# JiawangBian/SC-SfMLearner-Release

Hardware: AMD Instinct MI355X
Metric: train images/sec (+ warp-loss ms/step) KITTI 256x832 RN18 (higher is better)
Workload: dtype f32; 1 GPU; configs[1]: kitti 256x832, batch 12/GPU, 2 refs (seq 3), ResNet18 DispNet + ResNet18 PoseNet, ssim+mask+auto-mask, zeros padding, 1 scale; global_batch=12, parallelism=1 GPU, memory_format=contiguous (NCHW)

## Files before the change

### __graft_entry__.py

```python
import os
import sys

ROOT = os.path.dirname(os.path.abspath(__file__))
PKG = os.path.join(ROOT, "sc-sfmlearner-release_amd")
for p in (ROOT, PKG):
    if p not in sys.path:
        sys.path.insert(0, p)


REPORT_ORDER = ("dgrad", "vlog", "wrw", "decb", "enceval", "val", "dvis", "", "nets", "eval", "odom", "enc", "stem", "snip",
                "vis", "prep")


def build() -> None:
    from scsfm_hip import _lib, build as hip_build
    from scsfm_hip.libraries import BY_NAME, LATER, NEWER, ROWS
    libs = {row.name: _lib.CLib(hip_build.build_lib(row.name, force=False), row.header, row.abi, row.prefix)
            for row in ROWS}
    assert libs[""]._dll.scsfm_abi_version() == _lib.ABI_VERSION
    import inverse_warp
    import loss_functions
    import models
    from scsfm_hip import decoder, depth_eval, depth_vis, encoder, odometry, prepare, snippets, visualise
    from scsfm_hip import conv_wrw, decoder_bias, decoder_dgrad, encoder_eval, validation, validation_log
    from scsfm_hip import encoder_frozen, optim, training_state
    from oracle import scsfm_oracle
    for row in NEWER:
        print(f"[{row.tag}] {libs[row.name].path}: {len(libs[row.name].decls)} entry points resolved (ABI {row.abi})")
    for name in tuple(row.name for row in LATER) + REPORT_ORDER:
        print(f"[{BY_NAME[name].tag}] {libs[name].path}: {len(libs[name].decls)} entry points resolved")


def smoke() -> None:
    import torch

    import loss_functions as LF
    from oracle import scsfm_oracle as O
    from scsfm_hip import _lib, synth

    assert torch.cuda.is_available(), "smoke() needs a HIP device"
    lib = _lib.get()
    assert lib.path.endswith("libscsfm_hip.so")
    dev = torch.device("cuda:0")
    d = synth.make_batch(2, 128, 416, n_ref=2, seed=0, depth="smooth")

    def leaves(device):
        mv = lambda t: t.to(device).clone().requires_grad_(True)
        return ([mv(t) for t in d["tgt_depth"]], [[mv(t) for t in r] for r in d["ref_depths"]],
                [mv(p) for p in d["poses"]], [mv(p) for p in d["poses_inv"]])

    td, rd, ps, pi = leaves(dev)
    tgt, refs, K = d["tgt_img"].to(dev), [r.to(dev) for r in d["ref_imgs"]], d["intrinsics"].to(dev)
    photo, geom = LF.compute_photo_and_geometry_loss(tgt, refs, K, td, rd, ps, pi, 1, 1, 1, 1, "zeros")
    smooth = LF.compute_smooth_loss(td, tgt, rd, refs)
    (photo + 0.1 * smooth + 0.5 * geom).backward()
    torch.cuda.synchronize()

    td_c, rd_c, ps_c, pi_c = leaves("cpu")
    photo_c, geom_c = O.photo_and_geometry_loss(d["tgt_img"], d["ref_imgs"], d["intrinsics"], td_c, rd_c, ps_c, pi_c,
                                                1, 1, 1, 1, "zeros")
    smooth_c = O.smooth_loss(td_c, d["tgt_img"], rd_c, d["ref_imgs"])
    (photo_c + 0.1 * smooth_c + 0.5 * geom_c).backward()
    for name, a, b in (("photo", photo, photo_c), ("geom", geom, geom_c), ("smooth", smooth, smooth_c)):
        err = abs(float(a) - float(b))
        print(f"[smoke] {name}: hip {float(a):.7f} oracle {float(b):.7f} |d| {err:.2e}")
        assert err <= 1e-5, name
    pairs = [("g_tgt_depth", td[0].grad, td_c[0].grad), ("g_ref0_depth", rd[0][0].grad, rd_c[0][0].grad),
             ("g_ref1_depth", rd[1][0].grad, rd_c[1][0].grad), ("g_pose0", ps[0].grad, ps_c[0].grad),
             ("g_pose_inv1", pi[1].grad, pi_c[1].grad)]
    for name, a, b in pairs:
        scale = float(b.abs().max())
        bad = ((a.cpu() - b).abs() > 0.01 * scale).double().mean().item()
        print(f"[smoke] {name}: scale {scale:.3e} share of entries off by >1% of scale {bad:.2e}")
        assert bad <= 2e-3, name
    import torch.nn as nn
    from scsfm_hip import encoder as E
    assert _lib.get_stem().path.endswith("libscsfm_stem.so")
    xs = torch.randn(2, 4, 6, 8, device=dev)
    bn_a, bn_b = nn.BatchNorm2d(4).to(dev).train(), nn.BatchNorm2d(4).to(dev).train()
    f0, pooled = E.bn_act(xs, bn_a, pool=True)
    f0_ref = E.bn_act(xs, bn_b)
    assert torch.equal(f0, f0_ref) and torch.equal(pooled, E.max_pool(f0_ref))
    print("[smoke] stem: fused BatchNorm / ReLU / max-pool equals the separate ops")
    import numpy as np
    from scsfm_hip import visualise as V
    assert _lib.get_vis().path.endswith("libscsfm_vis.so")
    ramp = torch.linspace(0.05, 12.0, 70).reshape(2, 5, 7)
    for cmap, max_value in (("bone", None), ("rainbow", 10)):
        got = V.colourise(ramp.to(dev), colormap=cmap, max_value=max_value).cpu().numpy()
        table = V.colour_table(cmap)
        r = ramp.numpy()
        d = r.reshape(2, -1).max(axis=1)[:, None, None] if max_value is None else np.float32(max_value)
        xa = (r / d).astype(np.float32) * np.float32(len(table))
        want = table[np.clip(xa.astype(np.int64), 0, len(table) - 1)]
        assert got.shape == (2, 5, 7, 4) and np.array_equal(got, want), cmap
    print("[smoke] vis: bone and rainbow pictures of a ramp equal the table lookup")
    from scsfm_hip import depth_vis as DV
    assert _lib.get_dvis().path.endswith("libscsfm_dvis.so")
    depth = torch.linspace(0.5, 80.0, 35).reshape(5, 7)
    rng_, pics = DV.depth_pictures([depth.to(dev)])
    inv = 1 / (depth.numpy() + np.float32(1e-6))
    vmin, vmax = float(inv.min()), float(np.percentile(inv, 95))
    assert rng_.cpu().numpy().tolist() == [[vmin, vmax]]
    v = ((inv.astype(np.float64) - vmin).astype(np.float32).astype(np.float64) / (vmax - vmin)).astype(np.float32)
    xa = v * np.float32(256)
    want = DV.MAGMA[np.where(xa >= 256, 255, np.clip(xa, 0, 255).astype(np.int64))]
    assert pics[0].shape == (5, 7, 3) and np.array_equal(pics[0].cpu().numpy(), want)
    print("[smoke] dvis: the magma picture of a depth ramp equals the table lookup")
    from scsfm_hip import validation as VA
    assert _lib.get_val().path.endswith("libscsfm_val.so")
    f32 = np.float32
    rng = np.random.default_rng(0)
    gt_v = rng.uniform(0.05, 90.0, (2, 20, 60)).astype(f32)
    disp_v = rng.uniform(0.01, 1.5, (2, 10, 30)).astype(f32)
    res = VA.depth_errors(torch.from_numpy(gt_v).to(dev), torch.from_numpy(disp_v).to(dev), "kitti", is_disp=True)
    got = VA.batch_mean(res)
    y1, y2, x1, x2 = int(0.40810811 * 20), int(0.99189189 * 20), int(0.03594771 * 60), int(0.96405229 * 60)
    want = np.zeros(6)
    for g, dsp in zip(gt_v, disp_v):
        p = (f32(1) / dsp)[np.arange(20) // 2][:, np.arange(60) // 2]
        ok = np.zeros((20, 60), bool)
        ok[y1:y2, x1:x2] = True
        ok &= (g > f32(0.1)) & (g < f32(80))
        g, p = g[ok], np.clip(p[ok], f32(1e-3), f32(80))
        p = p * np.sort(g)[(g.size - 1) // 2] / np.sort(p)[(p.size - 1) // 2]
        t = np.maximum(g / p, p / g)
        e = np.abs(g - p).astype(np.float64)
        want += [e.mean(), (e / g).mean(), (e * e / g).mean(), (t < 1.25).mean(), (t < 1.25 ** 2).mean(),
                 (t < 1.25 ** 3).mean()]
    want /= 2
    print(f"[smoke] val: abs_rel hip {got[1]:.7f} numpy {want[1]:.7f}; a1 hip {got[3]:.7f} numpy {want[3]:.7f}")
    assert res.count.cpu().numpy().min() > 100 and np.allclose(got, want, rtol=1e-6, atol=0), (got, want)
    table = VA.ValidationTable(4, dev)
    rows_v = [(0.25, 0.002, 1.5), (0.5, float("nan"), 0.75), (0.125, 0.004, 0.25)]
    for i, vals_v in zip((0, 1, 3), rows_v):
        table.add_losses(i, *torch.tensor(vals_v, device=dev))
    mean_v, n_v = table.finish()
    sums_v = [0.0] * 4
    for p_v, s_v, g_v in rows_v:
        sums_v = [a + float(f32(b)) for a, b in zip(sums_v, (p_v, p_v, s_v, g_v))]
    want_v = [s / 3 for s in sums_v] + [0.0] * 3
    print(f"[smoke] val: table of 3 present rows of 4: photo {mean_v[1]:.7f} host {want_v[1]:.7f}, smooth {mean_v[2]} "
          f"(a NaN row), geometry {mean_v[3]:.7f} host {want_v[3]:.7f}")
    assert n_v == 3 and np.isnan(mean_v[2]) and mean_v[:2] + mean_v[3:] == want_v[:2] + want_v[3:], (mean_v, want_v)
    import torch.nn.functional as F
    from scsfm_hip import encoder_eval as EE
    assert _lib.get_enceval().path.endswith("libscsfm_enceval.so")
    bn_e = nn.BatchNorm2d(4).to(dev)
    with torch.no_grad():
        bn_e.running_mean.copy_(torch.tensor([0.5, -1.0, 0.0, 2.0]))
        bn_e.running_var.copy_(torch.tensor([0.25, 1.0, 4.0, 0.5]))
        bn_e.weight.copy_(torch.tensor([1.0, -0.5, 2.0, 0.0]))
        bn_e.bias.copy_(torch.tensor([0.0, 0.1, -0.2, 0.3]))
    bn_e.eval()
    with torch.no_grad():
        f0_e, pooled_e = EE.bn_act(xs, bn_e, pool=True)
        want_e = F.relu(bn_e(xs))
        assert torch.equal(f0_e, EE.bn_act(xs, bn_e)) and torch.equal(pooled_e, F.max_pool2d(f0_e, 3, 2, 1))
        assert torch.equal(pooled_e, EE.max_pool(f0_e))
    err_e = float((f0_e - want_e).abs().max())
    print(f"[smoke] enceval: eval-mode BatchNorm / ReLU / max-pool, max |fused - ATen| {err_e:.2e}")
    assert err_e <= 1e-5
    from scsfm_hip import decoder_bias as DB
    assert _lib.get_decb().path.endswith("libscsfm_decb.so")
    conv_b = nn.Conv2d(4, 3, 3).to(dev)
    xb = torch.randn(2, 4, 9, 11, device=dev)
    want_b = F.pad(F.elu(conv_b(xb)), (1, 1, 1, 1), mode="reflect")
    want_h = 10 * torch.sigmoid(conv_b(xb)) + 0.01
    (want_b.sum() + want_h.sum()).backward()
    want_gb = conv_b.bias.grad.clone()
    conv_b.bias.grad = None
    raw = F.conv2d(xb, conv_b.weight, None)
    got_b, got_h = DB.elu_pad(raw, conv_b.bias), DB.disp_head(raw, conv_b.bias, 10, 0.01)
    (got_b.sum() + got_h.sum()).backward()
    err_b = float((conv_b.bias.grad - want_gb).abs().max() / want_gb.abs().max())
    print(f"[smoke] decb: bias folded into elu_pad and disp_head, relative bias-gradient difference {err_b:.2e}")
    assert torch.equal(got_b, want_b) and float((got_h - want_h).abs().max()) <= 1e-6 and err_b <= 1e-5
    _smoke_wrw(dev)
    _smoke_vlog(dev)
    _smoke_dgrad(dev)
    _smoke_fbn(dev)
    _smoke_opt(dev)
    print("[smoke] ok")


def _smoke_opt(dev) -> None:
    import numpy as np
    import torch

    from scsfm_hip import _lib
    from scsfm_hip import optim as OP
    assert _lib.get_opt().path.endswith("libscsfm_opt.so")
    f32 = np.float32
    g = torch.Generator().manual_seed(7)
    shapes, lrs, wd, betas, eps = ((7,), (4, 6), (2 * OP.CHUNK + 3,), (3, 5, 5)), (1e-3, 1e-2), 0.01, (0.9, 0.999), 1e-8
    host = [torch.randn(s, generator=g) for s in shapes]
    params = [torch.nn.Parameter(t.to(dev)) for t in host]
    opt = OP.Adam([{"params": params[:2], "lr": lrs[0]}, {"params": params[2:], "lr": lrs[1]}], betas=betas, eps=eps,
                  weight_decay=wd)
    p = [t.numpy().copy() for t in host]
    m, v = [np.zeros_like(a) for a in p], [np.zeros_like(a) for a in p]
    b1c, b2, b2c, e, w = f32(1.0 - betas[0]), f32(betas[1]), f32(1.0 - betas[1]), f32(eps), f32(wd)
    for step in (1, 2, 3):
        grads = [torch.randn(s, generator=g) for s in shapes]
        for q, gr in zip(params, grads):
            q.grad = gr.to(dev)
        opt.step()
        for k, gr in enumerate(grads):
            step_size = f32(lrs[k // 2] / (1 - betas[0] ** step))
            bc2_sqrt = f32((1 - betas[1] ** step) ** 0.5)
            gk = gr.numpy() + w * p[k]
            m[k] = m[k] + b1c * (gk - m[k])
            v[k] = v[k] * b2 + (b2c * gk) * gk
            p[k] = p[k] - step_size * (m[k] / (np.sqrt(v[k]) / bc2_sqrt + e))
    state = opt.state_dict()["state"]
    for k in range(4):
        assert p[k].dtype == f32 and torch.equal(params[k].detach().cpu(), torch.from_numpy(p[k])), k
        assert torch.equal(state[k]["exp_avg"].cpu(), torch.from_numpy(m[k])), k
        assert torch.equal(state[k]["exp_avg_sq"].cpu(), torch.from_numpy(v[k])), k
        assert float(state[k]["step"]) == 3.0
    print("[smoke] opt: three Adam steps of four tensors in one launch each equal the numpy restatement bit for bit")


def _smoke_fbn(dev) -> None:
    import torch
    import torch.nn as nn
    import torch.nn.functional as F

    from scsfm_hip import _lib
    from scsfm_hip import encoder_frozen as EF
    assert _lib.get_fbn().path.endswith("libscsfm_fbn.so")
    g = torch.Generator().manual_seed(5)
    bn = nn.BatchNorm2d(4).to(dev)
    with torch.no_grad():
        bn.running_mean.copy_(torch.tensor([0.5, -1.0, 0.0, 2.0]))
        bn.running_var.copy_(torch.tensor([0.25, 1.0, 4.0, 0.5]))
        bn.weight.copy_(torch.tensor([1.0, -0.5, 2.0, 0.25]))
        bn.bias.copy_(torch.tensor([0.0, 0.1, -0.2, 0.3]))
    assert EF.freeze(bn) == 1 and not bn.train().training
    buffers = [b.clone() for b in bn.buffers()]
    x, identity = (torch.randn(2, 4, 6, 8, generator=g).to(dev).requires_grad_(True) for _ in range(2))
    gy = torch.randn(2, 4, 6, 8, generator=g).to(dev)
    leaves = (x, identity, bn.weight, bn.bias)
    y = EF.bn_act(x, bn, identity)
    got = torch.autograd.grad(y, leaves, gy)
    y_ref = F.relu(bn(x) + identity)
    want = torch.autograd.grad(y_ref, leaves, gy)
    err_y = float((y - y_ref).abs().max())
    err = max(float((a - b).abs().max() / b.abs().max()) for a, b in zip(got, want))
    print(f"[smoke] fbn: frozen BatchNorm / add / ReLU, max |fused - ATen| {err_y:.2e}, largest relative gradient "
          f"difference {err:.2e}")
    assert err_y <= 1e-5 and err <= 1e-5
    assert all(torch.equal(a, b) for a, b in zip(buffers, bn.buffers()))


def _smoke_wrw(dev) -> None:
    import torch
    import torch.nn.functional as F

    from scsfm_hip import _lib
    from scsfm_hip import conv_wrw as CW
    assert _lib.get_wrw().path.endswith("libscsfm_wrw.so")
    xw = torch.randn(2, 16, 7, 69, device=dev, requires_grad=True)
    ww = torch.randn(16, 16, 3, 3, device=dev, requires_grad=True)
    gy = torch.randn(2, 16, 5, 67, device=dev)
    gx_w, gw_w = torch.autograd.grad(CW.conv3x3_valid(xw, ww), (xw, ww), gy)
# ... 72 lines not shown
```

### sc-sfmlearner-release_amd/models/PoseResNet.py

```python
from __future__ import absolute_import, division, print_function

import torch
import torch.nn as nn

from .resnet_encoder import ResnetEncoder


class PoseDecoder(nn.Module):
    def __init__(self, num_ch_enc, num_input_features=1, num_frames_to_predict_for=1, stride=1):
        super().__init__()
        self.net = nn.ModuleList([
            nn.Conv2d(int(num_ch_enc[-1]), 256, 1),
            nn.Conv2d(num_input_features * 256, 256, 3, stride, 1),
            nn.Conv2d(256, 256, 3, stride, 1),
            nn.Conv2d(256, 6 * num_frames_to_predict_for, 1)])
        self.relu = nn.ReLU()

    def forward(self, input_features):
        out = torch.cat([self.relu(self.net[0](f[-1])) for f in input_features], 1)
        out = self.relu(self.net[1](out))
        out = self.relu(self.net[2](out))
        out = self.net[3](out)
        return 0.01 * out.mean(3).mean(2).view(-1, 6)


class PoseResNet(nn.Module):
    def __init__(self, num_layers=18, pretrained=True):
        super().__init__()
        self.encoder = ResnetEncoder(num_layers=num_layers, pretrained=pretrained, num_input_images=2)
        self.decoder = PoseDecoder(self.encoder.num_ch_enc)

    def init_weights(self):
        pass

    def forward(self, img1, img2):
        return self.decoder([self.encoder(torch.cat([img1, img2], 1))])
```

### sc-sfmlearner-release_amd/models/resnet_encoder.py

```python
from __future__ import absolute_import, division, print_function

import numpy as np
import torch
import torch.nn as nn


_encoder_ops = None


def _E():
    global _encoder_ops
    if _encoder_ops is None:
        from scsfm_hip import encoder
        _encoder_ops = encoder
    return _encoder_ops


_encoder_eval_ops = None


def _EV():
    global _encoder_eval_ops
    if _encoder_eval_ops is None:
        from scsfm_hip import encoder_eval
        _encoder_eval_ops = encoder_eval
    return _encoder_eval_ops


_encoder_frozen_ops = None


def _EF():
    global _encoder_frozen_ops
    if _encoder_frozen_ops is None:
        from scsfm_hip import encoder_frozen
        _encoder_frozen_ops = encoder_frozen
    return _encoder_frozen_ops


def _fused_applies(x, *bns):
    return x.is_cuda and _E().applies(x, *bns)


def _eval_applies(x, *bns):
    return x.is_cuda and _EV().applies(x, *bns)


def _frozen_applies(x, *bns, relu=True):
    return x.is_cuda and not any(bn.training for bn in bns) and _EF().applies(x, *bns, relu=relu)


def _bn_act(x, bn, act, identity=None):
    if _fused_applies(x, bn) and (identity is None or _fused_applies(identity)):
        return _E().bn_act(x, bn, identity, relu=act is not None)
    if _frozen_applies(x, bn, relu=act is not None) and (identity is None or _frozen_applies(identity)):
        return _EF().bn_act(x, bn, identity, relu=act is not None)
    if _eval_applies(x, bn) and (identity is None or _eval_applies(identity)):
        return _EV().bn_act(x, bn, identity, relu=act is not None)
    out = bn(x)
    if identity is not None:
        out = out + identity
    return out if act is None else act(out)


def _downsample(ds, x):
    return _bn_act(ds[0](x), ds[1], None)


def _conv3x3(cin, cout, stride=1):
    return nn.Conv2d(cin, cout, kernel_size=3, stride=stride, padding=1, bias=False)


class BasicBlock(nn.Module):
    expansion = 1

    def __init__(self, inplanes, planes, stride=1, downsample=None):
        super().__init__()
        self.conv1 = _conv3x3(inplanes, planes, stride)
        self.bn1 = nn.BatchNorm2d(planes)
        self.relu = nn.ReLU(inplace=True)
        self.conv2 = _conv3x3(planes, planes)
        self.bn2 = nn.BatchNorm2d(planes)
        self.downsample = downsample

    def forward(self, x):
        identity = x if self.downsample is None else _downsample(self.downsample, x)
        out = _bn_act(self.conv1(x), self.bn1, self.relu)
        return _bn_act(self.conv2(out), self.bn2, self.relu, identity)

    def forward_reference(self, x):
        identity = x if self.downsample is None else self.downsample(x)
        out = self.relu(self.bn1(self.conv1(x)))
        out = self.bn2(self.conv2(out))
        return self.relu(out + identity)


class Bottleneck(nn.Module):
    expansion = 4

    def __init__(self, inplanes, planes, stride=1, downsample=None):
        super().__init__()
        self.conv1 = nn.Conv2d(inplanes, planes, kernel_size=1, bias=False)
        self.bn1 = nn.BatchNorm2d(planes)
        self.conv2 = _conv3x3(planes, planes, stride)
        self.bn2 = nn.BatchNorm2d(planes)
        self.conv3 = nn.Conv2d(planes, planes * 4, kernel_size=1, bias=False)
        self.bn3 = nn.BatchNorm2d(planes * 4)
        self.relu = nn.ReLU(inplace=True)
        self.downsample = downsample

    def forward(self, x):
        identity = x if self.downsample is None else _downsample(self.downsample, x)
        out = _bn_act(self.conv1(x), self.bn1, self.relu)
        out = _bn_act(self.conv2(out), self.bn2, self.relu)
        return _bn_act(self.conv3(out), self.bn3, self.relu, identity)

    def forward_reference(self, x):
        identity = x if self.downsample is None else self.downsample(x)
        out = self.relu(self.bn1(self.conv1(x)))
        out = self.relu(self.bn2(self.conv2(out)))
        out = self.bn3(self.conv3(out))
        return self.relu(out + identity)


class ResNet(nn.Module):

    def __init__(self, block, layers, num_classes=1000, num_input_images=1):
        super().__init__()
        self.inplanes = 64
        self.conv1 = nn.Conv2d(num_input_images * 3, 64, kernel_size=7, stride=2, padding=3, bias=False)
        self.bn1 = nn.BatchNorm2d(64)
        self.relu = nn.ReLU(inplace=True)
        self.maxpool = nn.MaxPool2d(kernel_size=3, stride=2, padding=1)
        self.layer1 = self._make_layer(block, 64, layers[0])
        self.layer2 = self._make_layer(block, 128, layers[1], stride=2)
        self.layer3 = self._make_layer(block, 256, layers[2], stride=2)
        self.layer4 = self._make_layer(block, 512, layers[3], stride=2)
        self.avgpool = nn.AdaptiveAvgPool2d((1, 1))
        self.fc = nn.Linear(512 * block.expansion, num_classes)
        for m in self.modules():
            if isinstance(m, nn.Conv2d):
                nn.init.kaiming_normal_(m.weight, mode='fan_out', nonlinearity='relu')
            elif isinstance(m, nn.BatchNorm2d):
                nn.init.constant_(m.weight, 1)
                nn.init.constant_(m.bias, 0)

    def _make_layer(self, block, planes, blocks, stride=1):
        downsample = None
        if stride != 1 or self.inplanes != planes * block.expansion:
# ... 78 lines not shown
```

### sc-sfmlearner-release_amd/scsfm_hip/_lib.py

```python
from __future__ import annotations

import ctypes
import os
import re
import threading

import torch

from .libraries import BY_NAME, HERE, LATER, ROWS, SUMMARY, TABLE

__doc__ = (__doc__ or "") + SUMMARY + "\n"

HEADER = BY_NAME[""].header
LIB_PATH = os.environ.get("SCSFM_HIP_LIB") or BY_NAME[""].lib
ABI_VERSION = BY_NAME[""].abi

_CTYPES = {"int": ctypes.c_int, "unsigned": ctypes.c_uint, "size_t": ctypes.c_size_t, "double": ctypes.c_double,
           "float": ctypes.c_float}
_DECL = re.compile(r"^(int|size_t)\s+(scsfm_\w+)\s*\(([^)]*)\)\s*;", re.M | re.S)


def parse_header(path=HEADER):
    text = open(path).read()
    text = re.sub(r"/\*.*?\*/", "", text, flags=re.S)
    out = {}
    for ret, name, args in _DECL.findall(text):
        argtypes = []
        args = " ".join(args.split())
        if args and args != "void":
            for a in args.split(","):
                a = a.strip()
                if "*" in a:
                    argtypes.append(ctypes.c_void_p)
                else:
                    argtypes.append(_CTYPES[a.split()[0]])
        out[name] = (_CTYPES[ret], argtypes)
    return out


class ScsfmError(RuntimeError):
    pass


class CLib:

    def __init__(self, path, header=HEADER, abi=ABI_VERSION, prefix="scsfm_"):
        self.path = path
        self._dll = ctypes.CDLL(path)
        self.decls = parse_header(header)
        self._fn = {}
        self._prefix = prefix
        for name, (ret, argtypes) in self.decls.items():
            try:
                fn = getattr(self._dll, name)
            except AttributeError as e:
                raise ScsfmError(f"{path} does not export {name} (declared in {header})") from e
            fn.restype = ret
            fn.argtypes = argtypes
            self._fn[name] = fn
        if self._fn[prefix + "abi_version"]() != abi:
            raise ScsfmError(f"{path}: ABI version mismatch")

    def source_id(self):
        buf = ctypes.create_string_buffer(64)
        self._fn[self._prefix + "source_id"](buf, 64)
        return buf.value.decode()

    def call(self, name, *args):
        rc = self._fn[name](*args)
        if rc != 0:
            kind = "rejected argument" if rc == -1 else "hipError_t"
            raise ScsfmError(f"{name} failed with status {rc} ({kind})")

    def size(self, name, *args):
        return int(self._fn[name](*args))


_lock = threading.Lock()


def _load(row) -> CLib:
    from . import build as _build
    name = row.name
    path, own = (row.lib, True) if name else (LIB_PATH, "SCSFM_HIP_LIB" not in os.environ)
    if own and _build.lib_is_stale(name):
        have = _build.binary_source_id(path)
        try:
            _build.build_lib(name)
        except Exception as e:
            what = f"was built from other sources ({have}) than the tree's ({_build.lib_source_id(name)})" if have \
                else "is missing (or carries no source id)"
            raise ScsfmError(f"{path} {what} and cannot be built here: {e}") from e
    lib = CLib(path, row.header, row.abi, row.prefix)
    if own and lib.source_id() != _build.lib_source_id(name):
        raise ScsfmError(f"{path}: its source id {lib.source_id()} is not the tree's {_build.lib_source_id(name)}")
    return lib


def _getter(row):
    lib = None

    def get() -> CLib:
        nonlocal lib
        if lib is None:
            with _lock:
                if lib is None:
                    lib = _load(row)
        return lib
    get.__name__ = get.__qualname__ = f"get_{row.name}" if row.name else "get"
    get.__doc__ = f"""{os.path.basename(row.lib)} (one per process): {row.what} (include/{os.path.basename(row.header)}).
    Built in-tree with hipcc when it is missing or stale; raises when that is impossible (see ``_load``)."""
    return get


get = _getter(TABLE[0])
for _row in ROWS[1:]:
    globals().update({
        f"{_row.name.upper()}_HEADER": _row.header,
        f"{_row.name.upper()}_LIB_PATH": _row.lib,
        f"{_row.name.upper()}_ABI_VERSION": _row.abi,
        f"get_{_row.name}": _getter(_row),
    })
del _row
```

### sc-sfmlearner-release_amd/scsfm_hip/build.py

```python
from __future__ import annotations

import contextlib
import fcntl
import functools
import glob
import hashlib
import os
import shutil
import subprocess
import sys
import tempfile

from .libraries import BY_NAME, HERE, INCLUDE, LATER, ROWS, SUMMARY, TABLE, find

__doc__ = (__doc__ or "") + SUMMARY + "\n"

CSRC = BY_NAME[""].csrc
LIB = BY_NAME[""].lib
LOCK = LIB + ".lock"
LOG = LIB + ".buildlog"
ARCH = "gfx950"
FLAGS = ["-O3", "-std=c++17", "-fPIC", "-shared", f"--offload-arch={ARCH}", "-munsafe-fp-atomics",
         "-fno-gpu-rdc", "-Wall", "-Wno-unused-function",
         "-fno-slp-vectorize"]
ID_MARKER = b"scsfm-source-id:"


def lib_sources(name):
    return sorted(glob.glob(os.path.join(find(name).csrc, "*.hip")))


def lib_deps(name):
    row = find(name)
    return lib_sources(name) + sorted(glob.glob(os.path.join(row.csrc, "*.h"))) + [row.header]


def _hash(files, extra=()):
    h = hashlib.sha256()
    for path in files:
        h.update(os.path.basename(path).encode())
        h.update(open(path, "rb").read())
    h.update(" ".join(FLAGS).encode())
    if extra:
        h.update(b"\0extra:" + " ".join(extra).encode())
    return h.hexdigest()[:16]


def lib_source_id(name):
    return _hash(lib_deps(name))


def binary_source_id(path=LIB):
    try:
        blob = open(path, "rb").read()
    except OSError:
        return None
    i = blob.find(ID_MARKER)
    if i < 0:
        return None
    j = i + len(ID_MARKER)
    return blob[j:j + 16].decode("ascii", "replace")


def lib_is_stale(name):
    return binary_source_id(find(name).lib) != lib_source_id(name)


def build_lib(name, force=False, verbose=True):
    if not name:
        return build(force, verbose)
    return _build(find(name).lib, lib_source_id(name), lib_sources(name), ("-I", INCLUDE), force, verbose)



sources = functools.partial(lib_sources, "")
deps = functools.partial(lib_deps, "")
is_stale = functools.partial(lib_is_stale, "")


def source_id(extra=()):
    files = deps()
    if any("SCSFM_WITH_MARCH" in e or "variants" in e for e in extra):
        vsrc = os.path.join(os.path.dirname(os.path.dirname(HERE)), "variants", "src")
        files = files + sorted(p for p in glob.glob(os.path.join(vsrc, "*")) if os.path.isfile(p))
    return _hash(files, extra)


def build(force=False, verbose=True, extra=()):
    extra = tuple(extra)
    return _build(LIB, source_id(extra), sources(), extra, force, verbose)


for _row in ROWS[1:]:
    globals().update({
        f"{_row.name.upper()}_CSRC": _row.csrc,
        f"{_row.name.upper()}_LIB": _row.lib,
        f"{_row.name}_sources": functools.partial(lib_sources, _row.name),
        f"{_row.name}_deps": functools.partial(lib_deps, _row.name),
        f"{_row.name}_source_id": functools.partial(lib_source_id, _row.name),
        f"{_row.name}_is_stale": functools.partial(lib_is_stale, _row.name),
        f"build_{_row.name}": functools.partial(build_lib, _row.name),
    })
del _row


@contextlib.contextmanager
def _build_lock(lock=None):
    fd = os.open(lock or LOCK, os.O_CREAT | os.O_RDWR, 0o644)
    try:
        fcntl.flock(fd, fcntl.LOCK_EX)
        yield
    finally:
        try:
            fcntl.flock(fd, fcntl.LOCK_UN)
        finally:
            os.close(fd)


def _build(lib, want, srcs, extra, force, verbose):
    if not force and binary_source_id(lib) == want:
        return lib
    with _build_lock(lib + ".lock"):
        if not force and binary_source_id(lib) == want:
            return lib
        hipcc = shutil.which("hipcc") or "/opt/rocm/bin/hipcc"
        name = os.path.basename(lib)
        if not os.path.exists(hipcc):
            raise RuntimeError(f"hipcc not found: {name} cannot be built on this machine")
        fd, tmp = tempfile.mkstemp(prefix=name[:-len(".so")] + ".", suffix=f".{os.getpid()}.tmp", dir=HERE)
        os.close(fd)
        try:
            cmd = [hipcc, *FLAGS, f'-DSCSFM_SOURCE_ID="{want}"', *extra, "-o", tmp, *srcs]
            if verbose:
                print("[scsfm_hip.build]", " ".join(cmd), flush=True)
            subprocess.run(cmd, check=True)
            os.chmod(tmp, 0o755)
            os.replace(tmp, lib)
            with open(lib + ".buildlog", "a") as f:
                f.write(f"{want} {os.getpid()}\n")
        finally:
            if os.path.exists(tmp):
                os.unlink(tmp)
    return lib


if __name__ == "__main__":
    for _row in ROWS:
        build_lib(_row.name, force="--force" in sys.argv)
    for _row in ROWS:
        print(_row.lib)
```

### sc-sfmlearner-release_amd/scsfm_hip/config.py

```python
from __future__ import annotations

_hint = (1.0, 0.5)
_hint_dev = {}


def set_weight_hint(w_photo, w_geom):
    global _hint
    if w_photo is None:
        _hint = None
        return
    import numpy as np
    _hint = (float(np.float32(w_photo)), float(np.float32(w_geom)))
    for t in _hint_dev.values():
        t.copy_(t.new_tensor(_hint))


def weight_hint():
    return _hint


def hint_tensor(device):
    if _hint is None:
        return None
    import torch
# ... 8 lines not shown
def check_window():
    import os
    return os.environ.get("SCSFM_CHECK_WINDOW") == "1"


_smooth_rides = None


def smooth_rides_along():
    global _smooth_rides
    if _smooth_rides is None:
        import os
        _smooth_rides = os.environ.get("SCSFM_SMOOTH_RIDE", "1") != "0"
    return _smooth_rides


def set_smooth_rides_along(on):
    global _smooth_rides
    _smooth_rides = bool(on)


_errors_torch = None


def errors_on_torch():
    global _errors_torch
    if _errors_torch is None:
        import os
        _errors_torch = os.environ.get("SCSFM_ERRORS_TORCH", "0") == "1"
    return _errors_torch


def set_errors_on_torch(on):
    global _errors_torch
    _errors_torch = bool(on)


_decoder_bias = None


def decoder_bias_folded():
    global _decoder_bias
    if _decoder_bias is None:
        import os
        _decoder_bias = os.environ.get("SCSFM_DECODER_BIAS", "1") != "0"
    return _decoder_bias


def set_decoder_bias_folded(on):
    global _decoder_bias
    _decoder_bias = None if on is None else bool(on)


_decoder_wrw = None


def decoder_wrw():
    global _decoder_wrw
    if _decoder_wrw is None:
        import os
        _decoder_wrw = os.environ.get("SCSFM_DECODER_WRW", "1") != "0"
    return _decoder_wrw


def set_decoder_wrw(on):
    global _decoder_wrw
    _decoder_wrw = None if on is None else bool(on)


_decoder_dgrad = None


def decoder_dgrad():
    global _decoder_dgrad
    if _decoder_dgrad is None:
        import os
        _decoder_dgrad = os.environ.get("SCSFM_DECODER_DGRAD", "1") != "0"
    return _decoder_dgrad


def set_decoder_dgrad(on):
    global _decoder_dgrad
    _decoder_dgrad = None if on is None else bool(on)
```

### sc-sfmlearner-release_amd/scsfm_hip/libraries.py

```python
from __future__ import annotations

import os
from typing import NamedTuple

HERE = os.path.dirname(os.path.abspath(__file__))
INCLUDE = os.path.join(os.path.dirname(os.path.dirname(HERE)), "include")


class Library(NamedTuple):
    name: str
    abi: int
    tag: str
    what: str

    @property
    def csrc(self):
        return os.path.join(os.path.dirname(HERE), "csrc_" + self.name if self.name else "csrc")

    @property
    def header(self):
        return os.path.join(INCLUDE, f"scsfm_{self.name or 'hip'}.h")

    @property
    def lib(self):
        return os.path.join(HERE, f"libscsfm_{self.name or 'hip'}.so")

    @property
    def prefix(self):
        return f"scsfm_{self.name}_" if self.name else "scsfm_"


TABLE = (
    Library("", 9, "build", "the loss path"),
    Library("nets", 1, "build", "the depth decoder's fused glue"),
    Library("eval", 1, "build", "depth evaluation with median scaling"),
    Library("odom", 1, "build", "the pose chain of test_vo.py and KITTI odometry evaluation"),
    Library("enc", 1, "build", "the ResNet encoder's fused BatchNorm / ReLU / residual / max-pool glue"),
    Library("stem", 1, "build", "the ResNet stem's BatchNorm / ReLU fused with its max-pool"),
    Library("snip", 1, "build", "the 5-frame snippet pose evaluation of test_pose.py"),
    Library("prep", 1, "build:prep", "the resize and the Velodyne depth maps of data/prepare_train_data.py"),
    Library("vis", 1, "build:vis", "the input normalisation, the per-image maximum and the colour-mapped pictures of "
                                   "run_inference.py"),
    Library("dvis", 1, "build:dvis", "the scaled prediction, the colour range and the magma pictures of eval_depth.py "
                                     "--vis_dir"),
    Library("val", 2, "val:build", "the validation pass of train.py: the ground-truth metrics of --with-gt and the "
                                   "per-batch table of --shard-validation"),
    Library("enceval", 1, "enceval:build", "the ResNet encoder's eval-mode BatchNorm / ReLU / residual / max-pool glue"),
    Library("decb", 1, "decb:build", "the depth decoder's glue with the convolutions' biases folded in"),
    Library("wrw", 1, "wrw:build", "the weight gradient of the depth decoder's low-channel 3x3 convolutions"),
    Library("vlog", 1, "vlog:build", "the validation pictures of train.py --log-output"),
    Library("dgrad", 1, "dgrad:build", "the backward of the depth decoder's full-resolution tail"),
)
LATER = (
    Library("fbn", 1, "fbn:build", "the backward of the ResNet encoder's BatchNorm with frozen statistics (train.py "
                                   "--freeze-bn)"),
)
BY_NAME = {row.name: row for row in TABLE + LATER}
NEWER = (
    Library("opt", 1, "opt:build", "Adam over every parameter tensor in one launch (train.py --optimizer hip)"),
)
ROWS = TABLE + LATER + NEWER
_FIND = {row.name: row for row in ROWS}


def find(name):
    return _FIND[name]


SUMMARY = "\n".join(f"    {os.path.basename(row.lib):22s} {os.path.basename(row.csrc) + '/':14s} "
                    f"include/{os.path.basename(row.header):16s} {row.what}" for row in ROWS)
```

Baseline: 150.9 images/s.

## Add MFMA kernels for 1x1 downsample conv weight and stride-2 data gradients

```diff
diff --git a/__graft_entry__.py b/__graft_entry__.py
--- a/__graft_entry__.py
+++ b/__graft_entry__.py
@@ -14,18 +14,18 @@
 
 def build() -> None:
     from scsfm_hip import _lib, build as hip_build
-    from scsfm_hip.libraries import BY_NAME, LATER, NEWER, ROWS
+    from scsfm_hip.libraries import BY_NAME, EVERY, LATER, NEWER, NEWEST
     libs = {row.name: _lib.CLib(hip_build.build_lib(row.name, force=False), row.header, row.abi, row.prefix)
-            for row in ROWS}
+            for row in EVERY}
     assert libs[""]._dll.scsfm_abi_version() == _lib.ABI_VERSION
     import inverse_warp
     import loss_functions
     import models
     from scsfm_hip import decoder, depth_eval, depth_vis, encoder, odometry, prepare, snippets, visualise
     from scsfm_hip import conv_wrw, decoder_bias, decoder_dgrad, encoder_eval, validation, validation_log
-    from scsfm_hip import encoder_frozen, optim, training_state
+    from scsfm_hip import conv1x1, encoder_frozen, optim, training_state
     from oracle import scsfm_oracle
-    for row in NEWER:
+    for row in NEWER + NEWEST:
         print(f"[{row.tag}] {libs[row.name].path}: {len(libs[row.name].decls)} entry points resolved (ABI {row.abi})")
     for name in tuple(row.name for row in LATER) + REPORT_ORDER:
         print(f"[{BY_NAME[name].tag}] {libs[name].path}: {len(libs[name].decls)} entry points resolved")
@@ -181,7 +181,44 @@
     _smoke_dgrad(dev)
     _smoke_fbn(dev)
     _smoke_opt(dev)
+    _smoke_pw(dev)
     print("[smoke] ok")
+
+
+def _smoke_pw(dev) -> None:
+    import torch
+    import torch.nn.functional as F
+
+    from scsfm_hip import _lib
+    from scsfm_hip import conv1x1 as PW
+    assert _lib.get_pw().path.endswith("libscsfm_pw.so")
+    g = torch.Generator().manual_seed(9)
+    xp = torch.randn(2, 64, 7, 11, generator=g).to(dev).requires_grad_(True)
+    wp = (torch.randn(128, 64, 1, 1, generator=g) / 8).to(dev).requires_grad_(True)
+    gy = torch.randn(2, 128, 4, 6, generator=g).to(dev)
+    old = torch.backends.cudnn.deterministic, torch.backends.cudnn.benchmark
+    torch.backends.cudnn.deterministic, torch.backends.cudnn.benchmark = True, False
+    try:
+        y, y_ref = PW.conv1x1(xp, wp, None, 2), F.conv2d(xp, wp, None, 2)
+    finally:
+        torch.backends.cudnn.deterministic, torch.backends.cudnn.benchmark = old
+    assert torch.equal(y, y_ref)
+    gx_w, gw_w = PW.data_grad(gy, wp.detach(), 7, 11), PW.weight_grad(xp.detach(), gy, 2)
+    gx_m, gw_m = torch.autograd.grad(y_ref, (xp, wp), gy)
+    x64, w64 = (t.detach().double().requires_grad_(True) for t in (xp, wp))
+    gx_64, gw_64 = torch.autograd.grad(F.conv2d(x64, w64, None, 2), (x64, w64), gy.double())
+    xa, wa = (t.detach().double().abs().requires_grad_(True) for t in (xp, wp))
+    sx_64, sw_64 = torch.autograd.grad(F.conv2d(xa, wa, None, 2), (xa, wa), gy.double().abs())
+    u8 = 8 * 2.0 ** -24
+    for name, got, miopen, want, s in (("weight", gw_w, gw_m, gw_64, sw_64), ("data", gx_w, gx_m, gx_64, sx_64)):
+        err, err_m = (got - want).abs(), float((miopen - want).abs().max())
+        print(f"[smoke] pw: {name} gradient of a 64 -> 128 stride-2 1x1 convolution, max |hip - fp64| "
+              f"{float(err.max()):.2e} (MIOpen's {err_m:.2e})")
+        assert bool((err <= 2 * err_m + u8 * s).all()), name
+    assert bool((gx_w[:, :, 1::2, :] == 0).all()) and bool((gx_w[:, :, :, 1::2] == 0).all())
+    if (64, 128, 2) in PW.ROUTED and (64, 128, 2) in PW.ROUTED_DGRAD:
+        gx_f, gw_f = torch.autograd.grad(y, (xp, wp), gy)
+        assert torch.equal(gx_f, gx_w) and torch.equal(gw_f, gw_w)
 
 
 def _smoke_opt(dev) -> None:
diff --git a/include/scsfm_pw.h b/include/scsfm_pw.h
--- /dev/null
+++ b/include/scsfm_pw.h
@@ -0,0 +1,27 @@
+#ifndef SCSFM_PW_H_
+#define SCSFM_PW_H_
+
+#include <stddef.h>
+
+#ifndef SCSFM_ERR_ARG
+#define SCSFM_ERR_ARG (-1)
+#endif
+
+#ifdef __cplusplus
+extern "C" {
+#endif
+
+int scsfm_pw_abi_version(void);
+int scsfm_pw_source_id(char* buf, size_t n);
+int scsfm_pw_covers(int Cin, int Cout, int stride);
+size_t scsfm_pw_wrw_ws_bytes(int B, int Cin, int Cout, int H, int W, int stride);
+int scsfm_pw_wrw_f32(int B, int Cin, int Cout, int H, int W, int stride, const float* x, const float* dy, float* dw,
+                     void* ws, size_t ws_bytes, void* stream);
+int scsfm_pw_dgrad_f32(int B, int Cin, int Cout, int H, int W, const float* dy, const float* w, float* dx,
+                       void* stream);
+
+#ifdef __cplusplus
+}
+#endif
+
+#endif
diff --git a/sc-sfmlearner-release_amd/csrc_pw/scsfm_pointwise.hip b/sc-sfmlearner-release_amd/csrc_pw/scsfm_pointwise.hip
--- /dev/null
+++ b/sc-sfmlearner-release_amd/csrc_pw/scsfm_pointwise.hip
@@ -0,0 +1,290 @@
+#include <hip/hip_runtime.h>
+
+#include "scsfm_pw.h"
+
+#ifndef SCSFM_WRW_F32X4
+typedef float f32x4 __attribute__((ext_vector_type(4)));
+#endif
+
+namespace scsfm_pw {
+
+constexpr int kWave = 64;
+constexpr int kWaves = 4;
+constexpr int kThreads = kWave * kWaves;
+constexpr int kTM = 128, kTN = 64;
+constexpr int kKP = 32;
+constexpr int kSP = kKP + 2;
+constexpr int kSlots = 512;
+constexpr int kSlices = 8, kPerBlock = kThreads / kSlices;
+constexpr int kDM = 64, kDN = 64;
+constexpr int kKC = 32;
+constexpr int kSD = 80;
+
+__host__ __device__ inline int imin(int a, int b) { return a < b ? a : b; }
+__host__ __device__ inline int ceil_div(int a, int b) { return (a + b - 1) / b; }
+
+static __global__ __launch_bounds__(kThreads, 2) void wrw_kernel(int Cin, int Cout, int H, int W, int Wo, int HoWo,
+                                                                 int s, int chunks_img, int nchunks, int tiles_n,
+                                                                 const float* __restrict__ x,
+                                                                 const float* __restrict__ dy, float* __restrict__ ws) {
+  __shared__ float smem[(kTM + kTN) * kSP];
+  float* const ds = smem;
+  float* const xs = smem + kTM * kSP;
+  constexpr int ND = kTM / 8, NX = kTN / 8;
+
+  const int tid = threadIdx.x, lane = tid & (kWave - 1), wave = tid >> 6;
+  const int l15 = lane & 15, quad = lane >> 4;
+  const int q32 = tid & 31, r8 = tid >> 5;
+  const int P = gridDim.x, g = blockIdx.x;
+  const int co0 = (blockIdx.y / tiles_n) * kTM, ci0 = (blockIdx.y % tiles_n) * kTN;
+  const int HW = H * W;
+
+  f32x4 acc[2][4];
+#pragma unroll
+  for (int m = 0; m < 2; ++m)
+#pragma unroll
+    for (int c = 0; c < 4; ++c) acc[m][c] = f32x4{0.f, 0.f, 0.f, 0.f};
+
+  float pd[ND], px[NX];
+  auto prefetch = [&](int t) {
+    const int n = t / chunks_img, p = (t - n * chunks_img) * kKP + q32;
+    const bool in = p < HoWo;
+    const int y = p / Wo, xx = p - y * Wo;
+    const float* __restrict__ dg = dy + ((size_t)n * Cout + co0 + r8) * HoWo + p;
+    const float* __restrict__ xg = x + ((size_t)n * Cin + ci0 + r8) * HW + (s * y) * W + s * xx;
+#pragma unroll
+    for (int j = 0; j < ND; ++j) pd[j] = in ? dg[j * 8 * HoWo] : 0.f;
+#pragma unroll
+    for (int j = 0; j < NX; ++j) px[j] = in ? xg[j * 8 * HW] : 0.f;
+  };
+  auto commit = [&]() {
+#pragma unroll
+    for (int j = 0; j < ND; ++j) ds[(r8 + 8 * j) * kSP + q32] = pd[j];
+#pragma unroll
+    for (int j = 0; j < NX; ++j) xs[(r8 + 8 * j) * kSP + q32] = px[j];
+  };
+
+  const float* __restrict__ ap = ds + (wave * 32 + l15) * kSP + quad;
+  const float* __restrict__ bp = xs + l15 * kSP + quad;
+  if (g < nchunks) prefetch(g);
+  for (int t = g; t < nchunks; t += P) {
+    __syncthreads();
+    commit();
+    __syncthreads();
+    if (t + P < nchunks) prefetch(t + P);
+#pragma unroll
+    for (int k = 0; k < kKP / 4; ++k) {
+      float a[2], b[4];
+#pragma unroll
+      for (int m = 0; m < 2; ++m) a[m] = ap[m * 16 * kSP + 4 * k];
+#pragma unroll
+      for (int c = 0; c < 4; ++c) b[c] = bp[c * 16 * kSP + 4 * k];
+#pragma unroll
+      for (int m = 0; m < 2; ++m)
+#pragma unroll
+        for (int c = 0; c < 4; ++c) acc[m][c] = __builtin_amdgcn_mfma_f32_16x16x4f32(a[m], b[c], acc[m][c], 0, 0, 0);
+    }
+  }
+
+  float* __restrict__ out = ws + (size_t)g * (Cout * Cin);
+#pragma unroll
+  for (int m = 0; m < 2; ++m)
+#pragma unroll
+    for (int c = 0; c < 4; ++c)
+#pragma unroll
+      for (int i = 0; i < 4; ++i)
+        out[(co0 + wave * 32 + m * 16 + quad * 4 + i) * Cin + ci0 + c * 16 + l15] = acc[m][c][i];
+}
+
+static __global__ __launch_bounds__(kThreads) void sum_kernel(int G, int E, const float* __restrict__ ws,
+                                                              float* __restrict__ dw) {
+  __shared__ double part[kSlices][kPerBlock];
+  const int j = threadIdx.x & (kPerBlock - 1), sl = threadIdx.x / kPerBlock;
+  const int e = blockIdx.x * kPerBlock + j;
+  double s = 0.0;
+  if (e < E) {
+#pragma unroll 8
+    for (int g = sl; g < G; g += kSlices) s += (double)ws[(unsigned)g * (unsigned)E + (unsigned)e];
+  }
+  part[sl][j] = s;
+  __syncthreads();
+  if (sl == 0 && e < E) {
+    double t = part[0][j];
+#pragma unroll
+    for (int p = 1; p < kSlices; ++p) t += part[p][j];
+    dw[e] = (float)t;
+  }
+}
+
+static __global__ __launch_bounds__(kThreads, 2) void dgrad_kernel(int Cin, int Cout, int H, int W, int Wo, int HoWo,
+                                                                   int npix, const float* __restrict__ dy,
+                                                                   const float* __restrict__ w, float* __restrict__ dx) {
+  __shared__ float smem[2 * kKC * kSD];
+  float* const wl = smem;
+  float* const dl = smem + kKC * kSD;
+  constexpr int NR = kKC / 4;
+
+  const int tid = threadIdx.x, lane = tid & (kWave - 1), wave = tid >> 6;
+  const int l15 = lane & 15, quad = lane >> 4;
+  const int c64 = tid & 63, r4 = tid >> 6;
+  const int gp0 = blockIdx.x * kDN, ci0 = blockIdx.y * kDM;
+  const int mb = 2 * (wave & 1), nb = 2 * (wave >> 1);
+  const int HW = H * W;
+
+  f32x4 acc[2][2];
+#pragma unroll
+  for (int m = 0; m < 2; ++m)
+#pragma unroll
+    for (int c = 0; c < 2; ++c) acc[m][c] = f32x4{0.f, 0.f, 0.f, 0.f};
+
+  const int gp = gp0 + c64;
+  const bool in = gp < npix;
+  const int n_l = gp / HoWo, p_l = gp - n_l * HoWo;
+  const float* __restrict__ wg = w + (size_t)r4 * Cin + ci0 + c64;
+  const float* __restrict__ dg = dy + ((size_t)n_l * Cout + r4) * HoWo + p_l;
+  float pw[NR], pd[NR];
+  auto prefetch = [&](int k0) {
+#pragma unroll
+    for (int j = 0; j < NR; ++j) pw[j] = wg[(k0 + 4 * j) * Cin];
+#pragma unroll
+    for (int j = 0; j < NR; ++j) pd[j] = in ? dg[(k0 + 4 * j) * HoWo] : 0.f;
+  };
+  auto commit = [&]() {
+#pragma unroll
+    for (int j = 0; j < NR; ++j) wl[(r4 + 4 * j) * kSD + c64] = pw[j];
+#pragma unroll
+    for (int j = 0; j < NR; ++j) dl[(r4 + 4 * j) * kSD + c64] = pd[j];
+  };
+
+  const float* __restrict__ ap = wl + quad * kSD + mb * 16 + l15;
+  const float* __restrict__ bp = dl + quad * kSD + nb * 16 + l15;
+  prefetch(0);
+  for (int k0 = 0; k0 < Cout; k0 += kKC) {
+    __syncthreads();
+    commit();
+    __syncthreads();
+    if (k0 + kKC < Cout) prefetch(k0 + kKC);
+#pragma unroll
+    for (int k = 0; k < kKC / 4; ++k) {
+      float a[2], b[2];
+#pragma unroll
+      for (int m = 0; m < 2; ++m) a[m] = ap[4 * k * kSD + m * 16];
+#pragma unroll
+      for (int c = 0; c < 2; ++c) b[c] = bp[4 * k * kSD + c * 16];
+#pragma unroll
+      for (int m = 0; m < 2; ++m)
+#pragma unroll
+        for (int c = 0; c < 2; ++c) acc[m][c] = __builtin_amdgcn_mfma_f32_16x16x4f32(a[m], b[c], acc[m][c], 0, 0, 0);
+    }
+  }
+
+#pragma unroll
+  for (int c = 0; c < 2; ++c) {
+    const int q = gp0 + (nb + c) * 16 + l15;
+    if (q < npix) {
+      const int n = q / HoWo, p = q - n * HoWo;
+      const int y = p / Wo, xx = p - y * Wo;
+      const bool right = 2 * xx + 1 < W, below = 2 * y + 1 < H;
+      float* __restrict__ o = dx + ((size_t)n * Cin + ci0 + quad * 4) * HW + (2 * y) * W + 2 * xx;
+#pragma unroll
+      for (int m = 0; m < 2; ++m)
+#pragma unroll
+        for (int i = 0; i < 4; ++i) {
+          float* __restrict__ e = o + (m * 16 + mb * 16 + i) * HW;
+          e[0] = acc[m][c][i];
+          if (right) e[1] = 0.f;
+          if (below) {
+            e[W] = 0.f;
+            if (right) e[W + 1] = 0.f;
+          }
+        }
+    }
+  }
+}
+
+inline bool covers(int Cin, int Cout, int stride) {
+  return (Cin == 64 || Cin == 128 || Cin == 256 || Cin == 512) && (Cout == 128 || Cout == 256 || Cout == 512) &&
+         (stride == 1 || stride == 2);
+}
+
+struct Plan {
+  int Ho, Wo, HoWo, chunks_img, nchunks, tiles_n, tiles, P, E, npix;
+};
+
+inline bool plan_of(int B, int Cin, int Cout, int H, int W, int stride, Plan& p) {
+  if (B <= 0 || H <= 0 || W <= 0 || !covers(Cin, Cout, stride)) return false;
+  const long long lim = 1ll << 31;
+  p.Ho = (H - 1) / stride + 1;
+  p.Wo = (W - 1) / stride + 1;
+  if ((long long)B * Cin * H * W >= lim || (long long)p.Ho * p.Wo + kKP >= lim ||
+      (long long)B * Cout * p.Ho * p.Wo >= lim || (long long)B * p.Ho * p.Wo + kDN >= lim)
+    return false;
+  p.HoWo = p.Ho * p.Wo;
+  p.npix = B * p.HoWo;
+  p.chunks_img = ceil_div(p.HoWo, kKP);
+  p.nchunks = B * p.chunks_img;
+  if ((long long)B * p.chunks_img >= lim) return false;
+  p.tiles_n = Cin / kTN;
+  p.tiles = (Cout / kTM) * p.tiles_n;
+  p.P = imin(p.nchunks, kSlots / p.tiles);
+  p.E = Cout * Cin;
+  return true;
+}
+
+inline int launch_status() { return (int)hipGetLastError(); }
+
+}
+
+using namespace scsfm_pw;
+
+extern "C" {
+
+int scsfm_pw_abi_version(void) { return 1; }
+
+#ifndef SCSFM_SOURCE_ID
+#define SCSFM_SOURCE_ID "unknown"
+#endif
+static const char g_source_tag[] __attribute__((used)) = "scsfm-source-id:" SCSFM_SOURCE_ID;
+int scsfm_pw_source_id(char* buf, size_t n) {
+  const volatile char* id = g_source_tag + 16;
+  if (!buf || n == 0) return -1;
+  size_t i = 0;
+  for (; i + 1 < n && id[i]; ++i) buf[i] = id[i];
+  buf[i] = 0;
+  return 0;
+}
+
+int scsfm_pw_covers(int Cin, int Cout, int stride) { return covers(Cin, Cout, stride) ? 1 : 0; }
+
+size_t scsfm_pw_wrw_ws_bytes(int B, int Cin, int Cout, int H, int W, int stride) {
+  Plan p;
+  if (!plan_of(B, Cin, Cout, H, W, stride, p)) return 0;
+  return sizeof(float) * (size_t)p.P * p.E;
+}
+
+int scsfm_pw_wrw_f32(int B, int Cin, int Cout, int H, int W, int stride, const float* x, const float* dy, float* dw,
+                     void* ws, size_t ws_bytes, void* stream) {
+  Plan p;
+  if (!plan_of(B, Cin, Cout, H, W, stride, p) || !x || !dy || !dw || !ws || ((size_t)ws & 3) ||
+      ws_bytes < sizeof(float) * (size_t)p.P * p.E)
+    return SCSFM_ERR_ARG;
+  (void)hipGetLastError();
+  hipStream_t st = (hipStream_t)stream;
+  hipLaunchKernelGGL(wrw_kernel, dim3(p.P, p.tiles), dim3(kThreads), 0, st, Cin, Cout, H, W, p.Wo, p.HoWo, stride,
+                     p.chunks_img, p.nchunks, p.tiles_n, x, dy, (float*)ws);
+  if (const int rc = launch_status()) return rc;
+  hipLaunchKernelGGL(sum_kernel, dim3(ceil_div(p.E, kPerBlock)), dim3(kThreads), 0, st, p.P, p.E, (const float*)ws, dw);
+  return launch_status();
+}
+
+int scsfm_pw_dgrad_f32(int B, int Cin, int Cout, int H, int W, const float* dy, const float* w, float* dx,
+                       void* stream) {
+  Plan p;
+  if (!plan_of(B, Cin, Cout, H, W, 2, p) || !dy || !w || !dx) return SCSFM_ERR_ARG;
+  (void)hipGetLastError();
+  hipLaunchKernelGGL(dgrad_kernel, dim3(ceil_div(p.npix, kDN), Cin / kDM), dim3(kThreads), 0, (hipStream_t)stream, Cin,
+                     Cout, H, W, p.Wo, p.HoWo, p.npix, dy, w, dx);
+  return launch_status();
+}
+
+}
diff --git a/sc-sfmlearner-release_amd/models/PoseResNet.py b/sc-sfmlearner-release_amd/models/PoseResNet.py
--- a/sc-sfmlearner-release_amd/models/PoseResNet.py
+++ b/sc-sfmlearner-release_amd/models/PoseResNet.py
@@ -16,8 +16,14 @@
             nn.Conv2d(256, 6 * num_frames_to_predict_for, 1)])
         self.relu = nn.ReLU()
 
+    def _squeeze(self, x):
+        if x.is_cuda:
+            from scsfm_hip import conv1x1
+            return conv1x1.conv(self.net[0], x)
+        return self.net[0](x)
+
     def forward(self, input_features):
-        out = torch.cat([self.relu(self.net[0](f[-1])) for f in input_features], 1)
+        out = torch.cat([self.relu(self._squeeze(f[-1])) for f in input_features], 1)
         out = self.relu(self.net[1](out))
         out = self.relu(self.net[2](out))
         out = self.net[3](out)
diff --git a/sc-sfmlearner-release_amd/models/resnet_encoder.py b/sc-sfmlearner-release_amd/models/resnet_encoder.py
--- a/sc-sfmlearner-release_amd/models/resnet_encoder.py
+++ b/sc-sfmlearner-release_amd/models/resnet_encoder.py
@@ -63,8 +63,22 @@
     return out if act is None else act(out)
 
 
+_conv1x1_ops = None
+
+
+def _PW():
+    global _conv1x1_ops
+    if _conv1x1_ops is None:
+        from scsfm_hip import conv1x1
+        _conv1x1_ops = conv1x1
+    return _conv1x1_ops
+
+
 def _downsample(ds, x):
-    return _bn_act(ds[0](x), ds[1], None)
+    conv, bn = ds[0], ds[1]
+    hip = x.is_cuda and (bn.training or (_EF().is_frozen(bn) and _EF().enabled()))
+    y = _PW().conv(conv, x) if hip else conv(x)
+    return _bn_act(y, bn, None)
 
 
 def _conv3x3(cin, cout, stride=1):
diff --git a/sc-sfmlearner-release_amd/scsfm_hip/_lib.py b/sc-sfmlearner-release_amd/scsfm_hip/_lib.py
--- a/sc-sfmlearner-release_amd/scsfm_hip/_lib.py
+++ b/sc-sfmlearner-release_amd/scsfm_hip/_lib.py
@@ -7,7 +7,7 @@
 
 import torch
 
-from .libraries import BY_NAME, HERE, LATER, ROWS, SUMMARY, TABLE
+from .libraries import BY_NAME, EVERY, HERE, LATER, ROWS, SUMMARY, TABLE
 
 __doc__ = (__doc__ or "") + SUMMARY + "\n"
 
@@ -114,7 +114,7 @@
 
 
 get = _getter(TABLE[0])
-for _row in ROWS[1:]:
+for _row in EVERY[1:]:
     globals().update({
         f"{_row.name.upper()}_HEADER": _row.header,
         f"{_row.name.upper()}_LIB_PATH": _row.lib,
diff --git a/sc-sfmlearner-release_amd/scsfm_hip/build.py b/sc-sfmlearner-release_amd/scsfm_hip/build.py
--- a/sc-sfmlearner-release_amd/scsfm_hip/build.py
+++ b/sc-sfmlearner-release_amd/scsfm_hip/build.py
@@ -11,7 +11,7 @@
 import sys
 import tempfile
 
-from .libraries import BY_NAME, HERE, INCLUDE, LATER, ROWS, SUMMARY, TABLE, find
+from .libraries import BY_NAME, EVERY, HERE, INCLUDE, LATER, ROWS, SUMMARY, TABLE, find
 
 __doc__ = (__doc__ or "") + SUMMARY + "\n"
 
@@ -91,7 +91,7 @@
     return _build(LIB, source_id(extra), sources(), extra, force, verbose)
 
 
-for _row in ROWS[1:]:
+for _row in EVERY[1:]:
     globals().update({
         f"{_row.name.upper()}_CSRC": _row.csrc,
         f"{_row.name.upper()}_LIB": _row.lib,
@@ -145,7 +145,7 @@
 
 
 if __name__ == "__main__":
-    for _row in ROWS:
+    for _row in EVERY:
         build_lib(_row.name, force="--force" in sys.argv)
-    for _row in ROWS:
+    for _row in EVERY:
         print(_row.lib)
diff --git a/sc-sfmlearner-release_amd/scsfm_hip/config.py b/sc-sfmlearner-release_amd/scsfm_hip/config.py
--- a/sc-sfmlearner-release_amd/scsfm_hip/config.py
+++ b/sc-sfmlearner-release_amd/scsfm_hip/config.py
@@ -114,3 +114,19 @@
 def set_decoder_dgrad(on):
     global _decoder_dgrad
     _decoder_dgrad = None if on is None else bool(on)
+
+
+_conv1x1_bwd = None
+
+
+def conv1x1_bwd():
+    global _conv1x1_bwd
+    if _conv1x1_bwd is None:
+        import os
+        _conv1x1_bwd = os.environ.get("SCSFM_CONV1X1_BWD", "1") != "0"
+    return _conv1x1_bwd
+
+
+def set_conv1x1_bwd(on):
+    global _conv1x1_bwd
+    _conv1x1_bwd = None if on is None else bool(on)
diff --git a/sc-sfmlearner-release_amd/scsfm_hip/conv1x1.py b/sc-sfmlearner-release_amd/scsfm_hip/conv1x1.py
--- /dev/null
+++ b/sc-sfmlearner-release_amd/scsfm_hip/conv1x1.py
@@ -0,0 +1,115 @@
+from __future__ import annotations
+
+import torch
+import torch.nn.functional as F
+
+from . import _lib, config
+from .capi import _stream
+
+CIN = (64, 128, 256, 512)
+COUT = (128, 256, 512)
+STRIDES = (1, 2)
+ROUTED = {(64, 128, 2), (128, 256, 2), (256, 512, 2), (512, 256, 1)}
+ROUTED_DGRAD = {(64, 128, 2), (128, 256, 2), (256, 512, 2)}
+
+
+def covers(cin, cout, stride):
+    return int(cin) in CIN and int(cout) in COUT and int(stride) in STRIDES
+
+
+def dgrad_covers(cin, cout, stride):
+    return covers(cin, cout, stride) and int(stride) == 2
+
+
+def _triple(m):
+    return int(m.weight.shape[1]), int(m.weight.shape[0]), int(m.stride[0])
+
+
+def _plain1x1(x, m):
+    w, b = m.weight, m.bias
+    return (x.is_cuda and x.dtype == torch.float32 and x.dim() == 4 and x.is_contiguous() and x.numel() > 0
+            and w.is_cuda and w.dtype == torch.float32 and w.is_contiguous() and tuple(w.shape[2:]) == (1, 1)
+            and (b is None or (b.is_cuda and b.dtype == torch.float32))
+            and tuple(m.stride) in ((1, 1), (2, 2)) and tuple(m.padding) == (0, 0) and tuple(m.dilation) == (1, 1)
+            and m.groups == 1 and m.padding_mode == "zeros" and x.shape[1] == w.shape[1])
+
+
+def applies(x, m):
+    return bool(config.conv1x1_bwd() and torch.is_grad_enabled() and _plain1x1(x, m) and _triple(m) in ROUTED)
+
+
+def _out_size(n, stride):
+    return (n - 1) // stride + 1
+
+
+def weight_grad(x, gy, stride):
+    B, Cin, H, W = x.shape
+    Cout = gy.shape[1]
+    if not (x.is_cuda and gy.is_cuda and x.dtype == gy.dtype == torch.float32 and x.is_contiguous()
+            and gy.is_contiguous() and tuple(gy.shape) == (B, Cout, _out_size(H, stride), _out_size(W, stride))):
+        raise ValueError(f"scsfm_hip.conv1x1: CUDA fp32 contiguous x[B, Cin, H, W] and gy[B, Cout, Ho, Wo] only "
+                         f"(got {x.device} {x.dtype} {tuple(x.shape)} and {gy.device} {gy.dtype} {tuple(gy.shape)})")
+    lib = _lib.get_pw()
+    n = lib.size("scsfm_pw_wrw_ws_bytes", B, Cin, Cout, H, W, stride)
+    if n == 0:
+        raise ValueError(f"scsfm_hip.conv1x1: no kernel for {Cin} -> {Cout} channels, stride {stride}, at {B} x {H} x {W}")
+    ws = torch.empty(n // 4, dtype=torch.float32, device=x.device)
+    dw = torch.empty((Cout, Cin, 1, 1), dtype=torch.float32, device=x.device)
+    lib.call("scsfm_pw_wrw_f32", B, Cin, Cout, H, W, stride, x.data_ptr(), gy.data_ptr(), dw.data_ptr(), ws.data_ptr(),
+             n, _stream(x))
+    return dw
+
+
+def data_grad(gy, weight, H, W):
+    B, Cout = gy.shape[:2]
+    Cin = weight.shape[1]
+    if not (gy.is_cuda and weight.is_cuda and gy.dtype == weight.dtype == torch.float32 and gy.is_contiguous()
+            and weight.is_contiguous() and tuple(weight.shape) == (Cout, Cin, 1, 1) and dgrad_covers(Cin, Cout, 2)
+            and tuple(gy.shape) == (B, Cout, _out_size(H, 2), _out_size(W, 2))):
+        raise ValueError(f"scsfm_hip.conv1x1: CUDA fp32 contiguous gy[B, Cout, Ho, Wo] and weight[Cout, Cin, 1, 1] of a "
+                         f"covered stride-2 convolution only (got {gy.device} {gy.dtype} {tuple(gy.shape)} and "
+                         f"{weight.dtype} {tuple(weight.shape)} for {H} x {W})")
+    dx = torch.empty((B, Cin, H, W), dtype=torch.float32, device=gy.device)
+    _lib.get_pw().call("scsfm_pw_dgrad_f32", B, Cin, Cout, H, W, gy.data_ptr(), weight.data_ptr(), dx.data_ptr(),
+                       _stream(gy))
+    return dx
+
+
+class _Conv1x1(torch.autograd.Function):
+    @staticmethod
+    def forward(ctx, x, weight, bias, stride):
+        ctx.save_for_backward(x, weight)
+        ctx.stride = stride
+        ctx.bias_sizes = None if bias is None else [int(bias.shape[0])]
+        return F.conv2d(x, weight, bias, stride)
+
+    @staticmethod
+    def backward(ctx, gy):
+        x, weight = ctx.saved_tensors
+        s = ctx.stride
+        gy = gy.contiguous()
+        triple = (int(weight.shape[1]), int(weight.shape[0]), s)
+        gx = gw = gb = None
+
+        def aten(k):
+            mask = [k == 0, k == 1, k == 2]
+            return torch.ops.aten.convolution_backward(gy, x, weight, ctx.bias_sizes, [s, s], [0, 0], [1, 1], False,
+                                                       [0, 0], 1, mask)[k]
+
+        if ctx.needs_input_grad[0]:
+            gx = data_grad(gy, weight, x.shape[2], x.shape[3]) if triple in ROUTED_DGRAD else aten(0)
+        if ctx.needs_input_grad[1]:
+            gw = weight_grad(x, gy, s) if triple in ROUTED else aten(1)
+        if ctx.bias_sizes is not None and ctx.needs_input_grad[2]:
+            gb = aten(2)
+        return gx, gw, gb, None
+
+
+def conv1x1(x, weight, bias=None, stride=1):
+    return _Conv1x1.apply(x, weight, bias, int(stride))
+
+
+def conv(m, x):
+    if applies(x, m):
+        return conv1x1(x, m.weight, m.bias, int(m.stride[0]))
+    return m(x)
diff --git a/sc-sfmlearner-release_amd/scsfm_hip/libraries.py b/sc-sfmlearner-release_amd/scsfm_hip/libraries.py
--- a/sc-sfmlearner-release_amd/scsfm_hip/libraries.py
+++ b/sc-sfmlearner-release_amd/scsfm_hip/libraries.py
@@ -60,7 +60,11 @@
     Library("opt", 1, "opt:build", "Adam over every parameter tensor in one launch (train.py --optimizer hip)"),
 )
 ROWS = TABLE + LATER + NEWER
-_FIND = {row.name: row for row in ROWS}
+NEWEST = (
+    Library("pw", 1, "pw:build", "the weight and stride-2 data gradients of the encoders' 1x1 down-sample convolutions"),
+)
+EVERY = ROWS + NEWEST
+_FIND = {row.name: row for row in EVERY}
 
 
 def find(name):
@@ -68,4 +72,4 @@
 
 
 SUMMARY = "\n".join(f"    {os.path.basename(row.lib):22s} {os.path.basename(row.csrc) + '/':14s} "
-                    f"include/{os.path.basename(row.header):16s} {row.what}" for row in ROWS)
+                    f"include/{os.path.basename(row.header):16s} {row.what}" for row in EVERY)
```

Measured after the change: 153.7 images/s (median of 6 runs). 1.02x the previous value.
